# araffin/srl-zoo

Measured on AMD Instinct MI355X. Metric: images/sec (224x224x3) AE+VAE train step, higher is better.
Workload: dtype f32; 1 GPU; synthetic 224x224x3 obs, --losses autoencoder, custom_cnn, state-dim 200, bs=256 per GPU (512 frames fwd+bwd per step per GPU), Adam lr 0.005, normalised fp32 observations resident in HBM; global_batch=256, parallelism=dp1, rccl_ranks=1, devices=1

## Files before the change

include/srlz.h:

```cpp
#ifndef SRLZ_H
#define SRLZ_H

#include <stddef.h>
#include <stdint.h>

#ifdef __cplusplus
extern "C" {
#endif

typedef void* srlz_stream_t;

enum srlz_status {
  SRLZ_OK = 0,
  SRLZ_ERR_BAD_DESC = -1,
  SRLZ_ERR_WORKSPACE = -2,
  SRLZ_ERR_HIP = -3,
  SRLZ_ERR_NULL = -4
};

#define SRLZ_ABI_VERSION 104
int srlz_version(void);
const char* srlz_last_error(void);
int srlz_device_cus(void);

// ... 4 lines not shown
  int ksize;
  int stride;
  int pad;
  int transposed;
  int groups;
} srlz_conv64_desc;

size_t srlz_conv64_packed_floats(void);
int srlz_conv64_pack_weights(const float* w_ref, float* wpack_fwd, float* wpack_bwd,
                             const srlz_conv64_desc* d, srlz_stream_t stream);
int srlz_conv64_fwd_tiles(const srlz_conv64_desc* d);
int srlz_conv64_fwd(const float* x, const float* wpack_fwd, const float* bias, float* y, float* stats_partial,
                    const float* x_bnp, const srlz_conv64_desc* d, srlz_stream_t stream);
typedef struct {
  const float* y;
  const float* bnp;
  const float* sums;
  long long count;
  int training;
  float* dy_out;
} srlz_bn_bwd_operand;
int srlz_conv64_bwd_data(const float* dy, const float* wpack_bwd, float* dx, const srlz_bn_bwd_operand* dy_bn,
                         const srlz_conv64_desc* d, srlz_stream_t stream);
struct srlz_pool_desc_s;
int srlz_conv64_bwd_data_tiles(const srlz_conv64_desc* d);
int srlz_conv64_bwd_data_pool_sums(const float* dy, const float* wpack_bwd, float* dx, const float* pooled, const float* pool_bnp,
                                   const float* pool_y, const uint8_t* pool_argmax, const struct srlz_pool_desc_s* pd,
                                   float* bn_bwd_partial, const srlz_conv64_desc* d, srlz_stream_t stream);
int srlz_conv64_bwd_fused_supported(const srlz_conv64_desc* d);
int srlz_conv64_gather_pipe_supported(const srlz_conv64_desc* d, int backward_data);
int srlz_conv64_scatter_pipe_supported(const srlz_conv64_desc* d, int backward_data);
size_t srlz_conv64_bwd_fused_workspace(const srlz_conv64_desc* d);
int srlz_conv64_bwd_fused_bn_rows(const srlz_conv64_desc* d);
int srlz_conv64_bwd_fused_workgroups(const srlz_conv64_desc* d);
int srlz_conv64_bwd_fused(const float* x, const float* x_bnp, const float* dy, const srlz_bn_bwd_operand* dy_bn,
                          const float* wpack_bwd, float* dx, float* dw_ref, float* dbias ,
                          float* x_bn_bwd_partial , void* ws, size_t ws_bytes, const srlz_conv64_desc* d,
                          srlz_stream_t stream);
int srlz_conv64_wino_supported(const srlz_conv64_desc* d);
size_t srlz_conv64_wino_packed_floats(void);
int srlz_conv64_wino_pack_weights(const float* w_ref, float* upack_fwd, float* upack_bwd, srlz_stream_t stream);
int srlz_conv64_wino_tiles(const srlz_conv64_desc* d);
int srlz_conv64_wino_fwd(const float* x, const float* upack_fwd, const float* bias , float* y,
                         float* stats_partial , const float* x_bnp ,
                         const srlz_conv64_desc* d, srlz_stream_t stream);
int srlz_conv64_wino_bwd_data(const float* dy, const float* upack_bwd, float* dx, const srlz_conv64_desc* d, srlz_stream_t stream);
int srlz_conv64_wino_bwd_data_rows(const srlz_conv64_desc* d);
int srlz_conv64_wino_bwd_data_pool_sums(const float* dy, const float* upack_bwd, float* dx, const float* pooled, const float* pool_bnp,
                                        const float* pool_y, const uint8_t* pool_argmax, const struct srlz_pool_desc_s* pd,
                                        float* bn_bwd_partial, const srlz_conv64_desc* d, srlz_stream_t stream);
size_t srlz_conv64_wino_bwd_weight_workspace(const srlz_conv64_desc* d);
int srlz_conv64_wino_bwd_weight(const float* x, const float* dy, float* dw_ref, void* ws, size_t ws_bytes, const srlz_conv64_desc* d,
                                srlz_stream_t stream);
size_t srlz_conv64_bwd_weight_workspace(const srlz_conv64_desc* d);
int srlz_conv64_bwd_weight(const float* x, const float* dy, float* dw_ref, float* dbias, const float* x_bnp ,
                           const srlz_bn_bwd_operand* dy_bn ,
                           void* ws, size_t ws_bytes, const srlz_conv64_desc* d, srlz_stream_t stream);
int srlz_conv64_bwd_weight_plan(const srlz_conv64_desc* d, int has_x_bnp, int has_dy_bn, int out[4]);

typedef struct {
  int n, hi, wi, ho, wo;
  int cin, cout;
  int ksize, stride, pad;
  int groups;
} srlz_convn_desc;
size_t srlz_convn_packed_floats(const srlz_convn_desc* d);
int srlz_convn_pack_weights(const float* w_ref, float* wpack, const srlz_convn_desc* d, srlz_stream_t stream);
int srlz_convn_fwd_tiles(const srlz_convn_desc* d);
int srlz_convn_fwd(const float* x, const float* wpack, float* y, float* stats_partial, const float* x_bnp,
                   const srlz_convn_desc* d, srlz_stream_t stream);

typedef struct {
  int n;
  int c;
  int himg, wimg;
  int hf, wf;
  int kind;
  int groups;
} srlz_skinny_desc;

int srlz_skinny_tiles(const srlz_skinny_desc* d);
int srlz_conv1_workgroups(const srlz_skinny_desc* d);
int srlz_conv1_buffer_staging_supported(const srlz_skinny_desc* d);
int srlz_conv1_fwd(const float* x_nchw, const float* w_ref, float* y_nhwc, float* stats_partial,
                   const srlz_skinny_desc* d, srlz_stream_t stream);
int srlz_conv1_fwd_u8(const uint8_t* x_u8, const float* norm_lut, const float* w_ref, float* y_nhwc, float* stats_partial,
                      const srlz_skinny_desc* d, srlz_stream_t stream);
size_t srlz_skinny_bwd_weight_workspace(const srlz_skinny_desc* d);
int srlz_conv1_bwd_data(const float* dy_nhwc, const float* w_ref, float* dx_nchw, const srlz_skinny_desc* d,
                        srlz_stream_t stream);
int srlz_conv1_bwd_weight(const float* x_nchw, const float* dy_nhwc, float* dw_ref, void* ws, size_t ws_bytes,
                          const srlz_skinny_desc* d, srlz_stream_t stream);
int srlz_conv1_bwd_weight_fused(const float* x_nchw, const float* y_nhwc, const float* bnp, const uint8_t* argmax,
                                const float* dpooled, const float* sums, int training, float* dw_ref, void* ws,
                                size_t ws_bytes, const srlz_skinny_desc* d, const struct srlz_pool_desc_s* pd,
                                srlz_stream_t stream);
int srlz_conv1_bwd_weight_fused_u8(const uint8_t* x_u8, const float* norm_lut, const float* y_nhwc, const float* bnp,
                                   const uint8_t* argmax, const float* dpooled, const float* sums, int training, float* dw_ref,
                                   void* ws, size_t ws_bytes, const srlz_skinny_desc* d, const struct srlz_pool_desc_s* pd,
                                   srlz_stream_t stream);
int srlz_convT_out_fwd(const float* x_nhwc, const float* w_ref, const float* bias, float* y_nchw,
                       const float* x_bnp , const srlz_skinny_desc* d,
                       srlz_stream_t stream);
int srlz_convT_out_bwd_data(const float* dy_nchw, const float* w_ref, float* dx_nhwc, const float* x_raw,
                            const float* x_bnp, float* bn_bwd_partial, const srlz_skinny_desc* d, srlz_stream_t stream);
int srlz_convT_out_bwd_weight(const float* x_nhwc, const float* dy_nchw, float* dw_ref, float* dbias,
// ... 358 lines not shown
```

srl-zoo_amd/csrc/wino.hip:

```cpp
#include "common.h"

namespace {

typedef float f32x2 __attribute__((ext_vector_type(2)));
typedef unsigned u32x2 __attribute__((ext_vector_type(2)));

constexpr int WN_THREADS = 256;
constexpr int WN_TP = 32;
constexpr int WN_CHUNK = 16 * 4 * 64 * 4;
constexpr int WN_VCHUNK = 16 * 4 * WN_TP * 4;
constexpr int WN_VCOMP = 4 * WN_TP * 4;
constexpr unsigned WN_DROP = 0x80000000u;

struct WinoProg {
  int N, G;
  int H, W;
  int PA, PB;
  int ppi, ppg, tpg;
  unsigned mPPI, mPB;
  int sPPI, sPB;
  long long gstride;
};

__global__ void conv64_wino_pack_kernel(const float* __restrict__ w_ref, float* __restrict__ uf, float* __restrict__ ub) {
  const int id = blockIdx.x * blockDim.x + threadIdx.x;
  if (id >= 64 * 64) return;
  const int e = id & 3, m = (id >> 2) & 63, gq = (id >> 8) & 3, p = id >> 10;
  const int k = 16 * p + 4 * gq + e;
#pragma unroll
  for (int dir = 0; dir < 2; ++dir) {
    float* out = dir ? ub : uf;
    if (!out) continue;
    float gk[3][3];
#pragma unroll
    for (int ky = 0; ky < 3; ++ky)
#pragma unroll
      for (int kx = 0; kx < 3; ++kx)
        gk[ky][kx] = dir ? w_ref[((k * 64 + m) * 3 + (2 - ky)) * 3 + (2 - kx)] : w_ref[((m * 64 + k) * 3 + ky) * 3 + kx];
    float t[3][4];
#pragma unroll
    for (int ky = 0; ky < 3; ++ky) {
      t[ky][0] = gk[ky][0];
      t[ky][1] = 0.5f * (gk[ky][0] + gk[ky][1] + gk[ky][2]);
      t[ky][2] = 0.5f * (gk[ky][0] - gk[ky][1] + gk[ky][2]);
      t[ky][3] = gk[ky][2];
    }
#pragma unroll
    for (int nu = 0; nu < 4; ++nu) {
      const float u0 = t[0][nu];
      const float u1 = 0.5f * (t[0][nu] + t[1][nu] + t[2][nu]);
      const float u2 = 0.5f * (t[0][nu] - t[1][nu] + t[2][nu]);
      const float u3 = t[2][nu];
      const float u[4] = {u0, u1, u2, u3};
// ... 484 lines not shown
  const int wave = tid >> 6;
  const int q = lane >> 3, cpair = wave * 8 + (lane & 7);
  const int tw = (((q >> 2) * 2 + ((q >> 1) & 1)) * 64 + 2 * cpair) * 2 + (q & 1);
  const int ch = wave & 1, cq = wave >> 1, l31 = lane & 31, h = lane >> 5;
  const int tz = cq * 4 * WG_COMP + (h * 64 + 32 * ch + l31) * 2, tv = cq * 4 * WG_COMP + (h * 64 + l31) * 2;

  const long long tfl = (long long)P.N * P.H * P.W * 64;
  const __amdgpu_buffer_rsrc_t xb = raw_buffer(x - (P.W + 1) * 64, (unsigned)(tfl * 4) + (unsigned)(P.W + 1) * 256u);
  const __amdgpu_buffer_rsrc_t gb = raw_buffer(dy, (unsigned)(tfl * 4));

  f32x16 acc[4][2];
#pragma unroll
  for (int c = 0; c < 4; ++c)
#pragma unroll
    for (int b = 0; b < 2; ++b)
#pragma unroll
      for (int r = 0; r < 16; ++r) acc[c][b][r] = 0.f;

  const int s0 = slice * P.spw;
  int s1 = s0 + P.spw;
  if (s1 > P.stages) s1 = P.stages;
  WinoWgradRaw rw;
  WinoWgradPatch wp;
  if (s0 < s1) {
    wg_patch(wp, P, s0 * WG_SP + q, cpair);
    wg_request<S>(rw, wp, xb, gb, P.W);
    wg_land<S>(rw, smem + tw, smem + WG_OP + tw);
    wg_patch(wp, P, (s0 + 1) * WG_SP + q, cpair);
    wg_request<S>(rw, wp, xb, gb, P.W);
    for (int s = s0; s < s1; ++s) {
      const int par = (s - s0) & 1;
      float* cur = smem + par * 2 * WG_OP;
      float* nxt = smem + (par ^ 1) * 2 * WG_OP;
      __syncthreads();
      wg_land<S>(rw, nxt + tw, nxt + WG_OP + tw);
      wg_patch(wp, P, (s + 2) * WG_SP + q, cpair);
      wg_request<S>(rw, wp, xb, gb, P.W);
      __builtin_amdgcn_sched_barrier(0);
      wg_mfma_stage(acc, cur + tz, cur + WG_OP + tv);
    }
  }
  float* out = wpart + (size_t)blockIdx.x * (8 * 4096);
#pragma unroll
  for (int c = 0; c < 4; ++c)
#pragma unroll
    for (int b = 0; b < 2; ++b)
#pragma unroll
      for (int r = 0; r < 16; ++r) {
        const int co = 32 * ch + (r & 3) + 8 * (r >> 2) + 4 * h;
        out[((cq * 4 + c) * 64 + co) * 64 + 32 * b + l31] = acc[c][b][r];
      }
}

__global__ __launch_bounds__(256, 2) void conv64_wino_wgrad_kernel(const float* __restrict__ x, const float* __restrict__ dy,
                                                                   float* __restrict__ wpart, const WinoWgradProg P) {
  extern __shared__ __attribute__((aligned(16))) unsigned char smem_raw[];
  float* smem = (float*)smem_raw;
  const int xcd = blockIdx.x & 7, wi = blockIdx.x >> 3, wpx = gridDim.x >> 3;
  const int slice = xcd * (wpx >> 1) + (wi >> 1);
  if (wi & 1) wg_body<1>(x, dy, wpart, P, smem, slice);
  else wg_body<0>(x, dy, wpart, P, smem, slice);
}

__global__ __launch_bounds__(256) void conv64_wino_wgrad_reduce_a(const float* __restrict__ wpart, double* __restrict__ mid, int nwg, int per) {
  const int id = blockIdx.x * 256 + threadIdx.x;
  const int chunk = blockIdx.y;
  const int comp = id >> 12, rest = id & 4095;
  const int xi = comp >> 2, nu = comp & 3;
  const int half = nu >> 1, local = xi * 2 + (nu & 1);
  double t = 0.0;
  const int npair = nwg >> 1;
  for (int k = chunk * per; k < (chunk + 1) * per && k < npair; ++k) {
    const int b = ((k >> 3) * 2 + half) * 8 + (k & 7);
    t += (double)wpart[(size_t)b * (8 * 4096) + local * 4096 + rest];
  }
  mid[((size_t)chunk * 16 + comp) * 4096 + rest] = t;
}

__global__ __launch_bounds__(256) void conv64_wino_wgrad_reduce_b(const double* __restrict__ mid, int chunks, float* __restrict__ dw_ref) {
  __shared__ double m[16][17];
  const int comp = threadIdx.x >> 4, pr = threadIdx.x & 15;
  const int id = blockIdx.x * 16 + pr;
  double t = 0.0;
  for (int k = 0; k < chunks; ++k) t += mid[((size_t)k * 16 + comp) * 4096 + id];
  m[pr][comp] = t;
  __syncthreads();
  if (threadIdx.x < 144) {
    const int p2 = threadIdx.x / 9, tap = threadIdx.x - p2 * 9, ky = tap / 3, kx = tap - ky * 3;
    double r[4];
#pragma unroll
    for (int nu = 0; nu < 4; ++nu) {
      const double m0 = m[p2][nu], m1 = m[p2][4 + nu], m2 = m[p2][8 + nu], m3 = m[p2][12 + nu];
      r[nu] = ky == 0 ? m0 + 0.5 * (m1 + m2) : ky == 1 ? 0.5 * (m1 - m2) : 0.5 * (m1 + m2) + m3;
    }
    const double v = kx == 0 ? r[0] + 0.5 * (r[1] + r[2]) : kx == 1 ? 0.5 * (r[1] - r[2]) : 0.5 * (r[1] + r[2]) + r[3];
    dw_ref[(blockIdx.x * 16 + p2) * 9 + tap] = (float)v;
  }
}

constexpr int WG_CHUNKS = 8;

int wino_wgrad_program(WinoWgradProg* P, const srlz_conv64_desc* d, int* grid) {
  WinoProg F;
  if (wino_program(&F, d)) return 1;
  const long long total = (long long)d->n * F.ppi;
  if ((long long)d->n * d->hi * d->wi * 256 + (long long)(d->wi + 1) * 256 >= 0x7FFF0000LL || total + 64 >= (1LL << 31)) return 1;
  P->N = d->n; P->H = d->hi; P->W = d->wi; P->PA = F.PA; P->PB = F.PB; P->ppi = F.ppi;
  P->total = (int)total;
  P->stages = (int)((total + WG_SP - 1) / WG_SP);
  P->mPPI = F.mPPI; P->sPPI = F.sPPI; P->mPB = F.mPB; P->sPB = F.sPB;
  int g = 2 * srlz_device_cus();
  g = (g + 15) & ~15;
  while (g > 16 && (g >> 1) * 4 > P->stages) g -= 16;
  const int slices = g >> 1;
  P->spw = (P->stages + slices - 1) / slices;
  *grid = g;
  return 0;
}

}

extern "C" int srlz_conv64_wino_supported(const srlz_conv64_desc* d) {
  WinoProg P;
  return wino_program(&P, d) ? 0 : 1;
}

extern "C" size_t srlz_conv64_wino_packed_floats(void) { return (size_t)4 * WN_CHUNK; }

extern "C" int srlz_conv64_wino_pack_weights(const float* w_ref, float* upack_fwd, float* upack_bwd, srlz_stream_t stream) {
  SRLZ_REQUIRE(w_ref && (upack_fwd || upack_bwd), SRLZ_ERR_NULL, "conv64_wino_pack_weights: null pointer");
  SRLZ_LAUNCH(conv64_wino_pack_kernel, dim3(16), dim3(256), 0, as_stream(stream), w_ref, upack_fwd, upack_bwd);
  return 0;
}

extern "C" int srlz_conv64_wino_tiles(const srlz_conv64_desc* d) {
  WinoProg P;
  if (wino_program(&P, d)) return -1;
  return P.G * P.tpg;
}

static int wino_launch(const float* x, const float* upack, const float* bias, float* y, float* partial, const WinoProg& P,
                       const PoolSum* ps, const float* x_bnp, srlz_stream_t stream) {
  const int ntiles = P.G * P.tpg;
  int grid = 2 * srlz_device_cus();
  if (ntiles < grid) grid = ntiles;
  grid = (grid + 7) & ~7;
  const size_t lds = (size_t)2 * WN_VCHUNK * 4 + 2 * WN_TP * 4;
  const PoolSum none = SRLZ_NO_POOLSUM;
  hipStream_t st = as_stream(stream);
  if (ps) {
    SRLZ_MAX_LDS((conv64_wino_kernel<true, false>), lds);
    SRLZ_LAUNCH((conv64_wino_kernel<true, false>), dim3(grid), dim3(WN_THREADS), lds, st, x, upack, bias, y, partial, P, ntiles, *ps, x_bnp);
  } else if (x_bnp) {
    SRLZ_MAX_LDS((conv64_wino_kernel<false, true>), lds);
    SRLZ_LAUNCH((conv64_wino_kernel<false, true>), dim3(grid), dim3(WN_THREADS), lds, st, x, upack, bias, y, partial, P, ntiles, none, x_bnp);
  } else {
    SRLZ_MAX_LDS((conv64_wino_kernel<false, false>), lds);
    SRLZ_LAUNCH((conv64_wino_kernel<false, false>), dim3(grid), dim3(WN_THREADS), lds, st, x, upack, bias, y, partial, P, ntiles, none, x_bnp);
  }
  if (ps) {
    SRLZ_LAUNCH(conv64_wino_poolsum_zero_scale_kernel, dim3(WN_ZBLOCKS, P.G), dim3(256), 0, st, (const float*)y, *ps, partial, P.N, P.H,
                P.W, P.gstride, P.tpg + WN_ZBLOCKS, P.tpg);
  }
  return 0;
}

extern "C" int srlz_conv64_wino_bwd_data_rows(const srlz_conv64_desc* d) {
  WinoProg P;
  if (wino_program(&P, d)) return -1;
  return P.G * (P.tpg + WN_ZBLOCKS);
}

extern "C" int srlz_conv64_wino_fwd(const float* x, const float* upack, const float* bias, float* y, float* stats_partial,
                                    const float* x_bnp, const srlz_conv64_desc* d, srlz_stream_t stream) {
  SRLZ_REQUIRE(x && upack && y, SRLZ_ERR_NULL, "conv64_wino_fwd: null pointer");
  WinoProg P;
  SRLZ_REQUIRE(wino_program(&P, d) == 0, SRLZ_ERR_BAD_DESC,
               "conv64_wino_fwd: 3x3 stride 1 pad 1 on even sizes only (ask srlz_conv64_wino_supported)");
  return wino_launch(x, upack, bias, y, stats_partial, P, nullptr, x_bnp, stream);
}

extern "C" int srlz_conv64_wino_bwd_data(const float* dy, const float* upack_bwd, float* dx, const srlz_conv64_desc* d, srlz_stream_t stream) {
  SRLZ_REQUIRE(dy && upack_bwd && dx, SRLZ_ERR_NULL, "conv64_wino_bwd_data: null pointer");
  WinoProg P;
  SRLZ_REQUIRE(wino_program(&P, d) == 0, SRLZ_ERR_BAD_DESC,
               "conv64_wino_bwd_data: 3x3 stride 1 pad 1 on even sizes only (ask srlz_conv64_wino_supported)");
  return wino_launch(dy, upack_bwd, nullptr, dx, nullptr, P, nullptr, nullptr, stream);
}

extern "C" int srlz_conv64_wino_bwd_data_pool_sums(const float* dy, const float* upack_bwd, float* dx, const float* pooled,
                                                   const float* pool_bnp, const float* pool_y, const uint8_t* pool_argmax,
                                                   const srlz_pool_desc* pd, float* bn_bwd_partial, const srlz_conv64_desc* d,
                                                   srlz_stream_t stream) {
  SRLZ_REQUIRE(dy && upack_bwd && dx && pooled && pool_bnp && pool_y && pool_argmax && pd && bn_bwd_partial, SRLZ_ERR_NULL,
               "conv64_wino_bwd_data_pool_sums: null pointer");
  WinoProg P;
  SRLZ_REQUIRE(wino_program(&P, d) == 0, SRLZ_ERR_BAD_DESC,
               "conv64_wino_bwd_data_pool_sums: 3x3 stride 1 pad 1 on even sizes only (ask srlz_conv64_wino_supported)");
  SRLZ_REQUIRE(pd->n == d->n && pd->hp == d->hi && pd->wp == d->wi && !pd->out_nchw && (pd->groups > 1 ? pd->groups : 1) == P.G,
               SRLZ_ERR_BAD_DESC, "conv64_wino_bwd_data_pool_sums: the pooled map [%d,%d,%d] is not this layer's input [%d,%d,%d]", pd->n, pd->hp,
               pd->wp, d->n, d->hi, d->wi);
  const PoolSum ps = {pooled, pool_bnp, pool_y, pool_argmax, (long long)(pd->n / P.G) * pd->h * pd->w * 64, pd->h, pd->w, pd->pool_pad};
  return wino_launch(dy, upack_bwd, nullptr, dx, bn_bwd_partial, P, &ps, nullptr, stream);
}

extern "C" size_t srlz_conv64_wino_bwd_weight_workspace(const srlz_conv64_desc* d) {
  WinoWgradProg P;
  int grid;
  if (wino_wgrad_program(&P, d, &grid)) return 0;
  return (size_t)grid * 8 * 4096 * sizeof(float) + (size_t)WG_CHUNKS * 16 * 4096 * sizeof(double);
}

extern "C" int srlz_conv64_wino_bwd_weight(const float* x, const float* dy, float* dw_ref, void* ws, size_t ws_bytes,
                                           const srlz_conv64_desc* d, srlz_stream_t stream) {
  SRLZ_REQUIRE(x && dy && dw_ref && ws, SRLZ_ERR_NULL, "conv64_wino_bwd_weight: null pointer");
  WinoWgradProg P;
  int grid;
  SRLZ_REQUIRE(wino_wgrad_program(&P, d, &grid) == 0, SRLZ_ERR_BAD_DESC,
               "conv64_wino_bwd_weight: 3x3 stride 1 pad 1 on even sizes only (ask srlz_conv64_wino_supported)");
  const size_t part_bytes = (size_t)grid * 8 * 4096 * sizeof(float);
  SRLZ_REQUIRE(ws_bytes >= part_bytes + (size_t)WG_CHUNKS * 16 * 4096 * sizeof(double), SRLZ_ERR_WORKSPACE,
               "conv64_wino_bwd_weight: workspace too small (%zu bytes)", ws_bytes);
  hipStream_t st = as_stream(stream);
  const size_t lds = (size_t)4 * WG_OP * 4;
  SRLZ_MAX_LDS(conv64_wino_wgrad_kernel, lds);
  SRLZ_LAUNCH(conv64_wino_wgrad_kernel, dim3(grid), dim3(256), lds, st, x, dy, (float*)ws, P);
  double* mid = (double*)((char*)ws + part_bytes);
  const int npair = grid >> 1, per = (npair + WG_CHUNKS - 1) / WG_CHUNKS;
  SRLZ_LAUNCH(conv64_wino_wgrad_reduce_a, dim3(65536 / 256, WG_CHUNKS), dim3(256), 0, st, (const float*)ws, mid, grid, per);
  SRLZ_LAUNCH(conv64_wino_wgrad_reduce_b, dim3(256), dim3(256), 0, st, (const double*)mid, WG_CHUNKS, dw_ref);
  return 0;
}
```

srl-zoo_amd/srlz/_cabi.py:

```python
import ctypes
import os
from ctypes import c_int, c_longlong, c_ulonglong, c_float, c_double, c_void_p, c_size_t, c_char_p, POINTER, Structure

_HERE = os.path.dirname(os.path.abspath(__file__))
LIB_PATH = os.path.join(_HERE, "libsrlz_hip.so")


ABI_VERSION = 104


class SrlzError(RuntimeError):
    pass


class Conv64Desc(Structure):
    _fields_ = [("n", c_int), ("hi", c_int), ("wi", c_int), ("ho", c_int), ("wo", c_int), ("ksize", c_int),
                ("stride", c_int), ("pad", c_int), ("transposed", c_int), ("groups", c_int)]


class SkinnyDesc(Structure):
    _fields_ = [("n", c_int), ("c", c_int), ("himg", c_int), ("wimg", c_int), ("hf", c_int), ("wf", c_int),
                ("kind", c_int), ("groups", c_int)]


# ... 20 lines not shown


class InferBlockDesc(Structure):
    _fields_ = [("n", c_int), ("c_in", c_int), ("hi", c_int), ("wi", c_int), ("kind", c_int), ("pool_pad", c_int),
                ("out_nchw", c_int), ("stride_n", c_longlong), ("stride_c", c_longlong), ("stride_y", c_longlong),
                ("stride_x", c_longlong)]


INFER_IN, INFER_MID, INFER_LAST = 0, 1, 2


class InferDecDesc(Structure):
    _fields_ = [("n", c_int), ("c_in", c_int), ("c_out", c_int), ("hi", c_int), ("wi", c_int), ("kind", c_int), ("out_u8", c_int),
                ("bgr", c_int), ("in_stride_n", c_longlong), ("in_stride_c", c_longlong), ("in_stride_y", c_longlong),
                ("in_stride_x", c_longlong), ("out_stride_n", c_longlong), ("out_stride_c", c_longlong),
                ("out_stride_y", c_longlong), ("out_stride_x", c_longlong)]


INFER_DEC_FIRST, INFER_DEC_MID, INFER_DEC_OUT = 0, 1, 2

P = c_void_p
_BO = POINTER(BnBwdOperand)
_C64 = POINTER(Conv64Desc)
_SK = POINTER(SkinnyDesc)
_PD = POINTER(PoolDesc)
_CN = POINTER(ConvNDesc)
_IB = POINTER(InferBlockDesc)
_ID = POINTER(InferDecDesc)

_PROTOS = {
    "srlz_version": (c_int, []),
    "srlz_last_error": (c_char_p, []),
    "srlz_device_cus": (c_int, []),
    "srlz_conv64_packed_floats": (c_size_t, []),
    "srlz_conv64_pack_weights": (c_int, [P, P, P, _C64, P]),
    "srlz_conv64_fwd_tiles": (c_int, [_C64]),
    "srlz_conv64_fwd": (c_int, [P, P, P, P, P, P, _C64, P]),
    "srlz_conv64_bwd_data": (c_int, [P, P, P, _BO, _C64, P]),
    "srlz_conv64_bwd_weight_workspace": (c_size_t, [_C64]),
    "srlz_conv64_bwd_fused_supported": (c_int, [_C64]),
    "srlz_conv64_gather_pipe_supported": (c_int, [_C64, c_int]),
    "srlz_conv64_scatter_pipe_supported": (c_int, [_C64, c_int]),
    "srlz_conv64_bwd_fused_workspace": (c_size_t, [_C64]),
    "srlz_conv64_bwd_fused": (c_int, [P, P, P, _BO, P, P, P, P, P, P, c_size_t, _C64, P]),
    "srlz_conv64_bwd_fused_bn_rows": (c_int, [_C64]),
    "srlz_conv64_wino_supported": (c_int, [_C64]),
    "srlz_conv64_wino_packed_floats": (c_size_t, []),
    "srlz_conv64_wino_pack_weights": (c_int, [P, P, P, P]),
    "srlz_conv64_wino_tiles": (c_int, [_C64]),
    "srlz_conv64_wino_fwd": (c_int, [P, P, P, P, P, P, _C64, P]),
    "srlz_conv64_wino_bwd_data": (c_int, [P, P, P, _C64, P]),
    "srlz_conv64_wino_bwd_weight_workspace": (c_size_t, [_C64]),
    "srlz_conv64_wino_bwd_weight": (c_int, [P, P, P, P, c_size_t, _C64, P]),
    "srlz_conv64_wino_bwd_data_rows": (c_int, [_C64]),
    "srlz_conv64_wino_bwd_data_pool_sums": (c_int, [P, P, P, P, P, P, P, _PD, P, _C64, P]),
    "srlz_conv64_bwd_weight": (c_int, [P, P, P, P, P, _BO, P, c_size_t, _C64, P]),
    "srlz_conv64_bwd_weight_plan": (c_int, [_C64, c_int, c_int, POINTER(c_int)]),
    "srlz_conv64_bwd_fused_workgroups": (c_int, [_C64]),
    "srlz_conv1_workgroups": (c_int, [_SK]),
    "srlz_conv1_buffer_staging_supported": (c_int, [_SK]),
    "srlz_debug_conv1_fwd_generic": (c_int, [P, P, P, P, _SK, P]),
    "srlz_debug_conv1_fwd_u8_generic": (c_int, [P, P, P, P, P, _SK, P]),
    "srlz_debug_conv1_bwd_weight_fused_generic": (c_int, [P, P, P, P, P, P, c_int, P, P, c_size_t, _SK, _PD, P]),
    "srlz_debug_conv1_bwd_weight_fused_u8_generic": (c_int, [P, P, P, P, P, P, P, c_int, P, P, c_size_t, _SK, _PD, P]),
    "srlz_convT_out_os_plan": (c_int, [_SK, c_int, POINTER(c_int)]),
    "srlz_conv64_debug_program": (c_int, [_C64, c_int, POINTER(c_int), c_int]),
    "srlz_linear_debug_route": (c_int, [c_int, c_int, c_int, c_int, c_int, P, P, c_int, c_size_t, POINTER(c_int)]),
    "srlz_debug_placement": (c_int, [P, c_int, c_int, c_int, P]),
    "srlz_debug_mfma_peak": (c_int, [P, c_int, c_int, P]),
    "srlz_debug_mfma_valu": (c_int, [P, c_int, c_int, c_int, c_int, c_int, P]),
    "srlz_convn_packed_floats": (c_size_t, [_CN]),
    "srlz_convn_pack_weights": (c_int, [P, P, _CN, P]),
    "srlz_convn_fwd_tiles": (c_int, [_CN]),
    "srlz_convn_fwd": (c_int, [P, P, P, P, P, _CN, P]),
    "srlz_bn_finalize_chunks_workspace": (c_size_t, [c_int, c_int]),
    "srlz_bn_finalize_chunks": (c_int, [P, c_int, c_int, c_int, c_longlong, P, P, c_float, c_float, P, P, P, P, P, c_size_t, P]),
    "srlz_bn_eval_params_chunks": (c_int, [P, P, P, P, c_float, c_int, P, P]),
    "srlz_bn_add_relu": (c_int, [P, P, P, P, P, c_longlong, c_int, c_int, P]),
    "srlz_avgpool_nhwc": (c_int, [P, P, c_int, c_int, c_int, P]),
    "srlz_prelu_fwd": (c_int, [P, P, P, c_longlong, P]),
    "srlz_prelu_bwd": (c_int, [P, P, P, P, P, c_longlong, P]),
    "srlz_triplet_fwd": (c_int, [P, P, P, c_int, c_int, c_float, P, P, P]),
    "srlz_triplet_bwd": (c_int, [P, P, P, P, P, c_int, c_int, P, P, P, P]),
    "srlz_skinny_tiles": (c_int, [_SK]),
    "srlz_conv64_bwd_data_tiles": (c_int, [_C64]),
    "srlz_conv64_bwd_data_pool_sums": (c_int, [P, P, P, P, P, P, P, _PD, P, _C64, P]),
    "srlz_conv1_fwd": (c_int, [P, P, P, P, _SK, P]),
    "srlz_conv1_fwd_u8": (c_int, [P, P, P, P, P, _SK, P]),
    "srlz_conv1_bwd_weight_fused_u8": (c_int, [P, P, P, P, P, P, P, c_int, P, P, c_size_t, _SK, _PD, P]),
    "srlz_convT_out_fwd_loss_u8": (c_int, [P, P, P, P, P, P, P, P, P, _SK, P]),
    "srlz_normalize_lut": (c_int, [P, P]),
    "srlz_normalize_u8_planar": (c_int, [P, P, P, c_int, c_int, c_longlong, P]),
    "srlz_copy_frames_u8": (c_int, [P, P, c_longlong, P, P, c_longlong, c_int, c_longlong, P]),
    "srlz_copy_frames_u8_strided": (c_int, [P, P, c_longlong, c_longlong, c_longlong, P, P, c_longlong, c_longlong, c_longlong, c_int,
                                            c_longlong, P]),
    "srlz_occlude_frames_u8": (c_int, [P, P, c_longlong, P, P, P, c_int, c_int, c_int, c_int, P]),
    "srlz_skinny_bwd_weight_workspace": (c_size_t, [_SK]),
    "srlz_conv1_bwd_weight": (c_int, [P, P, P, P, c_size_t, _SK, P]),
    "srlz_conv1_bwd_data": (c_int, [P, P, P, _SK, P]),
    "srlz_conv1_bwd_weight_fused": (c_int, [P, P, P, P, P, P, c_int, P, P, c_size_t, _SK, _PD, P]),
    "srlz_bn_relu_pool_bwd_sums": (c_int, [P, P, P, P, P, P, P, P, P, c_size_t, _PD, P]),
    "srlz_convT_out_fwd": (c_int, [P, P, P, P, P, _SK, P]),
    "srlz_convT_out_bwd_data": (c_int, [P, P, P, P, P, P, _SK, P]),
    "srlz_bn_bwd_finalize_partials": (c_int, [P, c_int, c_int, P, P, P, P, c_size_t, P]),
    "srlz_convT_out_bwd_weight": (c_int, [P, P, P, P, P, P, c_size_t, _SK, P]),
    "srlz_convT_out_bwd_fused_supported": (c_int, [_SK]),
# ... 88 lines not shown
    "srlz_param_norms_grad": (c_int, [P, P, P, c_int, c_int, P, P, c_float, P]),
    "srlz_fold_grads": (c_int, [P, P, c_longlong, c_int, P]),
    "srlz_comm_unique_id_bytes": (c_size_t, []),
    "srlz_comm_unique_id": (c_int, [P]),
    "srlz_comm_init": (c_int, [P, c_int, c_int]),
    "srlz_comm_world": (c_int, []),
    "srlz_comm_allreduce_f32": (c_int, [P, c_longlong, P]),
    "srlz_comm_destroy": (c_int, []),
    "srlz_adam_step": (c_int, [P, P, P, P, c_longlong, c_double, c_double, c_double, c_double, c_int, c_float, P]),
    "srlz_adam_step_dev": (c_int, [P, P, P, P, c_longlong, c_double, c_double, c_double, c_double, P, P, c_float, P]),
    "srlz_infer_block_supported": (c_int, [_IB]),
    "srlz_infer_block_out_dims": (c_int, [_IB, POINTER(c_int), POINTER(c_int), POINTER(c_int), POINTER(c_int)]),
    "srlz_infer_tile": (c_int, []),
    "srlz_infer_packed_floats": (c_longlong, [c_int, c_int]),
    "srlz_infer_pack_weights": (c_int, [P, P, c_int, c_int, P]),
    "srlz_infer_block": (c_int, [P, P, P, P, P, _IB, P]),
    "srlz_infer_dec_supported": (c_int, [_ID]),
    "srlz_infer_dec_out_dims": (c_int, [_ID, POINTER(c_int), POINTER(c_int)]),
    "srlz_infer_dec_tile": (c_int, [c_int]),
    "srlz_infer_dec_packed_floats": (c_longlong, [c_int, c_int]),
    "srlz_infer_dec_pack_weights": (c_int, [P, P, c_int, c_int, P]),
    "srlz_infer_dec_block": (c_int, [P, P, P, P, P, _ID, P]),
    "srlz_infer_dec_out": (c_int, [P, P, P, P, _ID, P]),
    "srlz_rollout_supported": (c_int, [c_int, c_int, c_int, c_int]),
    "srlz_rollout_tile": (c_int, []),
    "srlz_rollout": (c_int, [P, P, c_longlong, P, P, P, P, P, P, P, P, P, P, P, P, c_int, c_int, c_int, c_int, c_int, c_int, c_int,
                             c_float, P]),
    "srlz_plan_supported": (c_int, [c_int, c_int, c_int, c_int, c_int, c_int]),
    "srlz_plan_workspace": (c_size_t, [c_int, c_int, c_int, c_int]),
    "srlz_plan_cem": (c_int, [P, P, P, P, P, P, P, P, P, P, c_longlong, P, P, P, P, P, P, c_size_t, c_int, c_int, c_int, c_int, c_int,
                              c_int, c_int, c_int, c_int, c_int, c_float, c_ulonglong, P]),
    "srlz_rollout_goal_supported": (c_int, [c_int, c_int, c_int, c_int, c_int]),
    "srlz_rollout_goal": (c_int, [P, P, c_longlong, P, P, P, P, P, P, P, P, P, P, P, P, c_int, c_int, c_int, c_int, c_int, c_int, c_int,
                                  c_float, P, c_longlong, c_float, c_int, P, P]),
    "srlz_plan_goal_supported": (c_int, [c_int, c_int, c_int, c_int, c_int, c_int, c_int]),
    "srlz_plan_goal_workspace": (c_size_t, [c_int, c_int, c_int, c_int]),
    "srlz_plan_cem_goal": (c_int, [P, P, P, P, P, P, P, P, P, P, c_longlong, P, P, P, P, P, P, c_size_t, c_int, c_int, c_int, c_int,
                                   c_int, c_int, c_int, c_int, c_int, c_int, c_float, c_ulonglong, P, c_longlong, c_float, c_int, P]),
    "srlz_beam_supported": (c_int, [c_int, c_int, c_int, c_int, c_int, c_int, c_int]),
    "srlz_beam_workspace": (c_size_t, [c_int, c_int, c_int, c_int, c_int]),
    "srlz_beam_leaves": (c_int, [c_int, c_int, c_int]),
    "srlz_beam_search": (c_int, [P, P, P, P, P, P, P, P, P, P, P, P, P, P, c_size_t, c_int, c_int, c_int, c_int, c_int, c_int, c_int,
                                 c_float, P, c_longlong, c_float, c_int, P]),
    "srlz_horizon_supported": (c_int, [c_int, c_int, c_int, c_int, c_int]),
    "srlz_horizon_rows": (c_int, [P, P, P, P, P, P, P, P, P, P, P, P, P, P, P, P, c_int, c_int, c_int, c_int, c_int, c_int, c_int, P]),
    "srlz_horizon_sums": (c_int, [P, P, P, P, P, P, c_int, c_int, P, P, P, P, P]),
}

_NOT_STATUS = {"srlz_version", "srlz_device_cus", "srlz_conv64_fwd_tiles", "srlz_skinny_tiles", "srlz_convn_fwd_tiles",
               "srlz_convT_out_bwd_fused_tiles", "srlz_convT_out_fwd_loss_workgroups", "srlz_conv64_bwd_fused_supported", "srlz_conv64_gather_pipe_supported",
               "srlz_conv64_scatter_pipe_supported",
               "srlz_convT_out_bwd_fused_supported",
               "srlz_conv64_bwd_data_tiles", "srlz_conv64_bwd_fused_bn_rows", "srlz_conv64_wino_supported", "srlz_conv64_wino_packed_floats",
               "srlz_conv64_wino_tiles", "srlz_conv64_wino_bwd_data_rows",
               "srlz_conv64_debug_program", "srlz_comm_world", "srlz_dense_supported",
               "srlz_dense_out_fwd_loss_workgroups", "srlz_reward_probe_chunk_rows", "srlz_infer_block_supported",
               "srlz_infer_tile", "srlz_conv64_bwd_fused_workgroups", "srlz_conv1_workgroups",
               "srlz_conv1_buffer_staging_supported", "srlz_infer_dec_supported", "srlz_infer_dec_tile", "srlz_rollout_supported",
               "srlz_rollout_tile", "srlz_plan_supported", "srlz_rollout_goal_supported", "srlz_plan_goal_supported",
               "srlz_horizon_supported", "srlz_beam_supported", "srlz_beam_leaves"}

EXPORTED = sorted(_PROTOS.keys())


def _load():
    if not os.path.exists(LIB_PATH):
        raise SrlzError(
            "libsrlz_hip.so not found at %s — build it with `python -c 'import __graft_entry__ as g; g.build()'` "
            "(or `make -C srl-zoo_amd/csrc`). There is no CPU fallback for the srl-zoo_amd hot path." % LIB_PATH)
    lib = ctypes.CDLL(LIB_PATH)
    for name, (res, args) in _PROTOS.items():
        fn = getattr(lib, name)
        fn.restype = res
        fn.argtypes = args
    got = lib.srlz_version()
    if got != ABI_VERSION:
        raise SrlzError("libsrlz_hip.so at %s reports ABI version %d, these bindings are written for %d (include/srlz.h "
                        "SRLZ_ABI_VERSION): rebuild with `make -C srl-zoo_amd/csrc`" % (LIB_PATH, got, ABI_VERSION))
    return lib


_lib = _load()


def error_text():
    return _lib.srlz_last_error().decode("utf-8", "replace")


_DEBUG_SYNC = bool(os.environ.get("SRLZ_SYNC"))


def _wrap(name):
    fn = getattr(_lib, name)
    if _PROTOS[name][0] is c_int and name not in _NOT_STATUS:
        def call(*a):
            rc = fn(*a)
            if rc != 0:
                raise SrlzError("%s failed (%d): %s" % (name, rc, error_text()))
            if _DEBUG_SYNC:
                import torch
                torch.cuda.synchronize()
            return rc
        call.__name__ = name
        return call
    return fn


# ... 14 lines not shown
```

Before: 45960 images/s.

## Fuse Winograd weight-grad split pair into one 512-thread workgroup with shared patch table

The old weight-gradient kernel ran two 256-thread workgroups per slice, each handling half of the Winograd components and each re-deriving patch addresses. The new default kernel merges them into one 512-thread workgroup: four waves transform x tiles and four waves transform dy tiles into shared LDS, one wave builds a small ring of patch-offset tables ahead of use, and every wave runs MFMA on both component halves. This aims to cut duplicate input loads, address arithmetic and launch count, and to overlap loads with MFMA through explicit scheduling barriers. The cost is more LDS per block and more accumulator registers, which may lower occupancy. The reduction kernel gains a flag for the new partial layout, and the old path stays available as a debug fallback when LDS opt-in is too small.

```diff
diff --git a/include/srlz.h b/include/srlz.h
--- a/include/srlz.h
+++ b/include/srlz.h
@@ -80,6 +80,9 @@
 size_t srlz_conv64_wino_bwd_weight_workspace(const srlz_conv64_desc* d);
 int srlz_conv64_wino_bwd_weight(const float* x, const float* dy, float* dw_ref, void* ws, size_t ws_bytes, const srlz_conv64_desc* d,
                                 srlz_stream_t stream);
+int srlz_debug_conv64_wino_bwd_weight_split(const float* x, const float* dy, float* dw_ref, void* ws, size_t ws_bytes,
+                                            const srlz_conv64_desc* d, srlz_stream_t stream);
+int srlz_debug_conv64_wino_bwd_weight_route(const srlz_conv64_desc* d);
 size_t srlz_conv64_bwd_weight_workspace(const srlz_conv64_desc* d);
 int srlz_conv64_bwd_weight(const float* x, const float* dy, float* dw_ref, float* dbias, const float* x_bnp ,
                            const srlz_bn_bwd_operand* dy_bn ,
diff --git a/srl-zoo_amd/csrc/wino.hip b/srl-zoo_amd/csrc/wino.hip
--- a/srl-zoo_amd/csrc/wino.hip
+++ b/srl-zoo_amd/csrc/wino.hip
@@ -1,4 +1,5 @@
 #include "common.h"
+#include <type_traits>
 
 namespace {
 
@@ -589,8 +590,8 @@
       }
 }
 
-__global__ __launch_bounds__(256, 2) void conv64_wino_wgrad_kernel(const float* __restrict__ x, const float* __restrict__ dy,
-                                                                   float* __restrict__ wpart, const WinoWgradProg P) {
+__global__ __launch_bounds__(256, 2) void conv64_wino_wgrad_split_kernel(const float* __restrict__ x, const float* __restrict__ dy,
+                                                                         float* __restrict__ wpart, const WinoWgradProg P) {
   extern __shared__ __attribute__((aligned(16))) unsigned char smem_raw[];
   float* smem = (float*)smem_raw;
   const int xcd = blockIdx.x & 7, wi = blockIdx.x >> 3, wpx = gridDim.x >> 3;
@@ -599,7 +600,222 @@
   else wg_body<0>(x, dy, wpart, P, smem, slice);
 }
 
-__global__ __launch_bounds__(256) void conv64_wino_wgrad_reduce_a(const float* __restrict__ wpart, double* __restrict__ mid, int nwg, int per) {
+typedef unsigned u32x4 __attribute__((ext_vector_type(4)));
+
+constexpr int W1_THREADS = 512;
+constexpr int W1_OP = 16 * WG_COMP;
+constexpr int W1_TSLOTS = 4;
+constexpr int W1_TENT = 12;
+constexpr size_t W1_LDS = (size_t)4 * W1_OP * 4 + (size_t)W1_TSLOTS * WG_SP * W1_TENT * 4;
+
+__device__ __forceinline__ void w1_table(unsigned* slot, const WinoWgradProg& P, int stage, int q) {
+  WinoWgradPatch wp;
+  wg_patch(wp, P, stage * WG_SP + q, 0);
+  u32x4* e = (u32x4*)(slot + q * W1_TENT);
+  e[0] = u32x4{wp.vtop, wp.vmid, wp.vbot, wp.vmid};
+  e[1] = u32x4{wp.lef ? wp.vtop : WN_DROP, wp.lef ? wp.vmid : WN_DROP, wp.lef ? wp.vbot : WN_DROP, WN_DROP};
+  e[2] = u32x4{wp.rig ? wp.vtop : WN_DROP, wp.rig ? wp.vmid : WN_DROP, wp.rig ? wp.vbot : WN_DROP, WN_DROP};
+}
+
+struct W1Entry { u32x4 m, l, r; };
+
+template <int ROLE>
+__device__ __forceinline__ void w1_entry(W1Entry& t, const unsigned* ent) {
+  if (ROLE == 0) { t.m = *(const u32x4*)ent; t.l = *(const u32x4*)(ent + 4); t.r = *(const u32x4*)(ent + 8); }
+  else t.m[1] = ent[1];
+}
+
+template <int ROLE>
+__device__ __forceinline__ void w1_request(f32x2 (&d)[ROLE == 0 ? 16 : 4], const W1Entry& t, unsigned cp8, __amdgpu_buffer_rsrc_t xb,
+                                           __amdgpu_buffer_rsrc_t gb, int W) {
+  if (ROLE == 0) {
+#pragma unroll
+    for (int r = 0; r < 4; ++r)
+#pragma unroll
+      for (int c = 0; c < 4; ++c) {
+        const u32x4 cls = c == 0 ? t.l : c == 3 ? t.r : t.m;
+        const unsigned off = (r == 0 ? cls[0] : r == 3 ? cls[2] : cls[1]) + cp8;
+        const u32x2 v = __builtin_amdgcn_raw_buffer_load_b64(xb, off + (unsigned)(c * 256), r * W * 256, 0);
+        d[r * 4 + c] = f32x2{__uint_as_float(v[0]), __uint_as_float(v[1])};
+      }
+  } else {
+    const unsigned off = t.m[1] + cp8;
+#pragma unroll
+    for (int i = 0; i < 2; ++i)
+#pragma unroll
+      for (int j = 0; j < 2; ++j) {
+        const u32x2 v = __builtin_amdgcn_raw_buffer_load_b64(gb, off + (unsigned)(j * 256), i * W * 256, 0);
+        d[i * 2 + j] = f32x2{__uint_as_float(v[0]), __uint_as_float(v[1])};
+      }
+  }
+}
+
+template <int ROLE>
+__device__ __forceinline__ void w1_land(const f32x2 (&d)[ROLE == 0 ? 16 : 4], float* __restrict__ Ow) {
+  int two = 2;
+  asm volatile("" : "+v"(two));
+  float* __restrict__ Ow1 = Ow + two;
+#pragma unroll
+  for (int S = 0; S < 2; ++S) {
+    f32x2 o[2][4];
+    if (ROLE == 0) {
+      f32x2 e[4][2];
+#pragma unroll
+      for (int r = 0; r < 4; ++r) {
+        if (S == 0) { e[r][0] = d[r * 4 + 0] - d[r * 4 + 2]; e[r][1] = d[r * 4 + 1] + d[r * 4 + 2]; }
+        else        { e[r][0] = d[r * 4 + 2] - d[r * 4 + 1]; e[r][1] = d[r * 4 + 1] - d[r * 4 + 3]; }
+      }
+#pragma unroll
+      for (int j = 0; j < 2; ++j) {
+        o[j][0] = e[0][j] - e[2][j]; o[j][1] = e[1][j] + e[2][j]; o[j][2] = e[2][j] - e[1][j]; o[j][3] = e[1][j] - e[3][j];
+      }
+    } else {
+      f32x2 t[2][2];
+#pragma unroll
+      for (int i = 0; i < 2; ++i) {
+        if (S == 0) { t[i][0] = d[i * 2]; t[i][1] = d[i * 2] + d[i * 2 + 1]; }
+        else        { t[i][0] = d[i * 2] - d[i * 2 + 1]; t[i][1] = -d[i * 2 + 1]; }
+      }
+#pragma unroll
+      for (int j = 0; j < 2; ++j) {
+        o[j][0] = t[0][j]; o[j][1] = t[0][j] + t[1][j]; o[j][2] = t[0][j] - t[1][j]; o[j][3] = -t[1][j];
+      }
+    }
+#pragma unroll
+    for (int ch = 0; ch < 2; ++ch)
+#pragma unroll
+      for (int j = 0; j < 2; ++j)
+#pragma unroll
+        for (int xi = 0; xi < 4; ++xi) (ch ? Ow1 : Ow)[(xi * 4 + 2 * S + j) * WG_COMP] = o[j][xi][ch];
+  }
+}
+
+struct W1Frag { f32x2 z[2][2], v[2][2]; };
+
+__device__ __forceinline__ void w1_read(W1Frag& f, const float* __restrict__ Zp, const float* __restrict__ Vp) {
+#pragma unroll
+  for (int j = 0; j < 2; ++j)
+#pragma unroll
+    for (int b = 0; b < 2; ++b) {
+      f.z[j][b] = *(const f32x2*)(Zp + j * 256 + b * 64);
+      f.v[j][b] = *(const f32x2*)(Vp + j * 256 + b * 64);
+    }
+}
+
+__device__ __forceinline__ void w1_mfma_comp(f32x16 (&acc)[2][2], const W1Frag& f) {
+#pragma unroll
+  for (int j = 0; j < 2; ++j)
+#pragma unroll
+    for (int e = 0; e < 2; ++e)
+#pragma unroll
+      for (int bo = 0; bo < 2; ++bo)
+#pragma unroll
+        for (int bi = 0; bi < 2; ++bi)
+          acc[bo][bi] = __builtin_amdgcn_mfma_f32_32x32x2f32(f.z[j][bo][e], f.v[j][bi][e], acc[bo][bi], 0, 0, 0);
+}
+
+template <int ROLE>
+__device__ __forceinline__ void w1_body(const float* __restrict__ x, const float* __restrict__ dy, float* __restrict__ wpart,
+                                        const WinoWgradProg& P, float* smem, int slice, int wave) {
+  const int tid = threadIdx.x;
+  int lane = tid & 63;
+  asm volatile("" : "+v"(lane));
+  const int q = lane >> 3, cpair = (wave & 3) * 8 + (lane & 7);
+  const unsigned cp8 = (unsigned)cpair * 8u;
+  const int tw = (ROLE == 0 ? W1_OP : 0) + (((q >> 2) * 2 + ((q >> 1) & 1)) * 64 + 2 * cpair) * 2 + (q & 1);
+  unsigned* tab = (unsigned*)(smem + 4 * W1_OP);
+  const bool builder = ROLE == 1 && wave == 4 && lane < WG_SP;
+  const int l31 = lane & 31, h = lane >> 5;
+  const int tm = wave * 2 * WG_COMP + (h * 64 + l31) * 2;
+
+  const long long tfl = (long long)P.N * P.H * P.W * 64;
+  const __amdgpu_buffer_rsrc_t xb = raw_buffer(x - (P.W + 1) * 64, (unsigned)(tfl * 4) + (unsigned)(P.W + 1) * 256u);
+  const __amdgpu_buffer_rsrc_t gb = raw_buffer(dy, (unsigned)(tfl * 4));
+
+  f32x16 acc[2][2][2];
+#pragma unroll
+  for (int c = 0; c < 2; ++c)
+#pragma unroll
+    for (int bo = 0; bo < 2; ++bo)
+#pragma unroll
+      for (int bi = 0; bi < 2; ++bi)
+#pragma unroll
+        for (int r = 0; r < 16; ++r) acc[c][bo][bi][r] = 0.f;
+
+  const int s0 = slice * P.spw;
+  int s1 = s0 + P.spw;
+  if (s1 > P.stages) s1 = P.stages;
+  if (s0 < s1) {
+    f32x2 raw[ROLE == 0 ? 16 : 4];
+    W1Entry te;
+    W1Frag f1;
+    if (builder) {
+#pragma unroll
+      for (int i = 0; i < 3; ++i) w1_table(tab + i * WG_SP * W1_TENT, P, s0 + i, lane);
+    }
+    __syncthreads();
+    w1_entry<ROLE>(te, tab + q * W1_TENT);
+    w1_request<ROLE>(raw, te, cp8, xb, gb, P.W);
+    w1_land<ROLE>(raw, smem + tw);
+    w1_entry<ROLE>(te, tab + (WG_SP + q) * W1_TENT);
+    w1_request<ROLE>(raw, te, cp8, xb, gb, P.W);
+    auto stage = [&](auto first, int s) {
+      constexpr bool FIRST = decltype(first)::value;
+      const int k = s - s0;
+      float* cur = smem + (k & 1) * 2 * W1_OP;
+      float* nxt = smem + ((k & 1) ^ 1) * 2 * W1_OP;
+      __syncthreads();
+      W1Frag f0;
+      w1_read(f0, cur + tm, cur + W1_OP + tm);
+      w1_entry<ROLE>(te, tab + (((k + 2) & (W1_TSLOTS - 1)) * WG_SP + q) * W1_TENT);
+      __builtin_amdgcn_sched_barrier(0);
+      if (ROLE == 1 && !FIRST) w1_mfma_comp(acc[1], f1);
+      w1_land<ROLE>(raw, nxt + tw);
+      w1_request<ROLE>(raw, te, cp8, xb, gb, P.W);
+      if (builder) w1_table(tab + ((k + 3) & (W1_TSLOTS - 1)) * WG_SP * W1_TENT, P, s + 3, lane);
+      if (ROLE == 0 && !FIRST) w1_mfma_comp(acc[1], f1);
+      __builtin_amdgcn_sched_barrier(0);
+      w1_read(f1, cur + tm + WG_COMP, cur + W1_OP + tm + WG_COMP);
+      w1_mfma_comp(acc[0], f0);
+#pragma unroll
+      for (int i = 0; i < 8; ++i) {
+        __builtin_amdgcn_sched_group_barrier(0x100, 1, 0);
+        __builtin_amdgcn_sched_group_barrier(0x008, 1, 0);
+      }
+      __builtin_amdgcn_sched_group_barrier(0x008, 8, 0);
+      __builtin_amdgcn_sched_barrier(0);
+    };
+    stage(std::true_type{}, s0);
+    for (int s = s0 + 1; s < s1; ++s) stage(std::false_type{}, s);
+    w1_mfma_comp(acc[1], f1);
+  }
+  float* out = wpart + (size_t)blockIdx.x * (16 * 4096) + (size_t)wave * (2 * 4096);
+#pragma unroll
+  for (int c = 0; c < 2; ++c)
+#pragma unroll
+    for (int bo = 0; bo < 2; ++bo)
+#pragma unroll
+      for (int bi = 0; bi < 2; ++bi)
+#pragma unroll
+        for (int r = 0; r < 16; ++r) {
+          const int co = 32 * bo + (r & 3) + 8 * (r >> 2) + 4 * h;
+          out[(c * 64 + co) * 64 + 32 * bi + l31] = acc[c][bo][bi][r];
+        }
+}
+
+__global__ __launch_bounds__(W1_THREADS, 2) void conv64_wino_wgrad_kernel(const float* __restrict__ x, const float* __restrict__ dy,
+                                                                          float* __restrict__ wpart, const WinoWgradProg P) {
+  extern __shared__ __attribute__((aligned(16))) unsigned char smem_raw[];
+  float* smem = (float*)smem_raw;
+  const int xcd = blockIdx.x & 7, wi = blockIdx.x >> 3, wpx = gridDim.x >> 3;
+  const int slice = xcd * wpx + wi;
+  const int wave = __builtin_amdgcn_readfirstlane(threadIdx.x >> 6);
+  if (wave < 4) w1_body<0>(x, dy, wpart, P, smem, slice, wave);
+  else w1_body<1>(x, dy, wpart, P, smem, slice, wave);
+}
+
+__global__ __launch_bounds__(256) void conv64_wino_wgrad_reduce_a(const float* __restrict__ wpart, double* __restrict__ mid, int nwg, int per,
+                                                                  int onepass) {
   const int id = blockIdx.x * 256 + threadIdx.x;
   const int chunk = blockIdx.y;
   const int comp = id >> 12, rest = id & 4095;
@@ -609,7 +825,7 @@
   const int npair = nwg >> 1;
   for (int k = chunk * per; k < (chunk + 1) * per && k < npair; ++k) {
     const int b = ((k >> 3) * 2 + half) * 8 + (k & 7);
-    t += (double)wpart[(size_t)b * (8 * 4096) + local * 4096 + rest];
+    t += (double)(onepass ? wpart[(size_t)k * (16 * 4096) + comp * 4096 + rest] : wpart[(size_t)b * (8 * 4096) + local * 4096 + rest]);
   }
   mid[((size_t)chunk * 16 + comp) * 4096 + rest] = t;
 }
@@ -653,6 +869,18 @@
   P->spw = (P->stages + slices - 1) / slices;
   *grid = g;
   return 0;
+}
+
+bool wino_wgrad_onepass(const WinoWgradProg& P, int grid) {
+  static int lds_optin = -1;
+  if (lds_optin < 0) {
+    int dev = 0, v = 0, w = 0;
+    if (hipGetDevice(&dev) != hipSuccess || hipDeviceGetAttribute(&v, hipDeviceAttributeMaxSharedMemoryPerBlock, dev) != hipSuccess) v = 0;
+    if (v && hipDeviceGetAttribute(&w, hipDeviceAttributeSharedMemPerBlockOptin, dev) != hipSuccess) w = 0;
+    (void)hipGetLastError();
+    lds_optin = v > w ? v : w;
+  }
+  return (size_t)lds_optin >= W1_LDS && (grid & 15) == 0 && P.stages > 0;
 }
 
 }
@@ -748,23 +976,46 @@
   return (size_t)grid * 8 * 4096 * sizeof(float) + (size_t)WG_CHUNKS * 16 * 4096 * sizeof(double);
 }
 
-extern "C" int srlz_conv64_wino_bwd_weight(const float* x, const float* dy, float* dw_ref, void* ws, size_t ws_bytes,
-                                           const srlz_conv64_desc* d, srlz_stream_t stream) {
-  SRLZ_REQUIRE(x && dy && dw_ref && ws, SRLZ_ERR_NULL, "conv64_wino_bwd_weight: null pointer");
+static int wino_wgrad_launch(const char* who, bool allow_onepass, const float* x, const float* dy, float* dw_ref, void* ws, size_t ws_bytes,
+                             const srlz_conv64_desc* d, srlz_stream_t stream) {
+  SRLZ_REQUIRE(x && dy && dw_ref && ws, SRLZ_ERR_NULL, "%s: null pointer", who);
   WinoWgradProg P;
   int grid;
   SRLZ_REQUIRE(wino_wgrad_program(&P, d, &grid) == 0, SRLZ_ERR_BAD_DESC,
-               "conv64_wino_bwd_weight: 3x3 stride 1 pad 1 on even sizes only (ask srlz_conv64_wino_supported)");
+               "%s: 3x3 stride 1 pad 1 on even sizes only (ask srlz_conv64_wino_supported)", who);
   const size_t part_bytes = (size_t)grid * 8 * 4096 * sizeof(float);
   SRLZ_REQUIRE(ws_bytes >= part_bytes + (size_t)WG_CHUNKS * 16 * 4096 * sizeof(double), SRLZ_ERR_WORKSPACE,
-               "conv64_wino_bwd_weight: workspace too small (%zu bytes)", ws_bytes);
+               "%s: workspace too small (%zu bytes)", who, ws_bytes);
   hipStream_t st = as_stream(stream);
-  const size_t lds = (size_t)4 * WG_OP * 4;
-  SRLZ_MAX_LDS(conv64_wino_wgrad_kernel, lds);
-  SRLZ_LAUNCH(conv64_wino_wgrad_kernel, dim3(grid), dim3(256), lds, st, x, dy, (float*)ws, P);
+  const int onepass = allow_onepass && wino_wgrad_onepass(P, grid) ? 1 : 0;
+  if (onepass) {
+    SRLZ_MAX_LDS(conv64_wino_wgrad_kernel, W1_LDS);
+    SRLZ_LAUNCH(conv64_wino_wgrad_kernel, dim3(grid >> 1), dim3(W1_THREADS), W1_LDS, st, x, dy, (float*)ws, P);
+  } else {
+    const size_t lds = (size_t)4 * WG_OP * 4;
+    SRLZ_MAX_LDS(conv64_wino_wgrad_split_kernel, lds);
+    SRLZ_LAUNCH(conv64_wino_wgrad_split_kernel, dim3(grid), dim3(256), lds, st, x, dy, (float*)ws, P);
+  }
   double* mid = (double*)((char*)ws + part_bytes);
   const int npair = grid >> 1, per = (npair + WG_CHUNKS - 1) / WG_CHUNKS;
-  SRLZ_LAUNCH(conv64_wino_wgrad_reduce_a, dim3(65536 / 256, WG_CHUNKS), dim3(256), 0, st, (const float*)ws, mid, grid, per);
+  SRLZ_LAUNCH(conv64_wino_wgrad_reduce_a, dim3(65536 / 256, WG_CHUNKS), dim3(256), 0, st, (const float*)ws, mid, grid, per, onepass);
   SRLZ_LAUNCH(conv64_wino_wgrad_reduce_b, dim3(256), dim3(256), 0, st, (const double*)mid, WG_CHUNKS, dw_ref);
   return 0;
 }
+
+extern "C" int srlz_conv64_wino_bwd_weight(const float* x, const float* dy, float* dw_ref, void* ws, size_t ws_bytes,
+                                           const srlz_conv64_desc* d, srlz_stream_t stream) {
+  return wino_wgrad_launch("conv64_wino_bwd_weight", true, x, dy, dw_ref, ws, ws_bytes, d, stream);
+}
+
+extern "C" int srlz_debug_conv64_wino_bwd_weight_split(const float* x, const float* dy, float* dw_ref, void* ws, size_t ws_bytes,
+                                                       const srlz_conv64_desc* d, srlz_stream_t stream) {
+  return wino_wgrad_launch("debug_conv64_wino_bwd_weight_split", false, x, dy, dw_ref, ws, ws_bytes, d, stream);
+}
+
+extern "C" int srlz_debug_conv64_wino_bwd_weight_route(const srlz_conv64_desc* d) {
+  WinoWgradProg P;
+  int grid;
+  if (wino_wgrad_program(&P, d, &grid)) return -1;
+  return wino_wgrad_onepass(P, grid) ? 1 : 0;
+}
diff --git a/srl-zoo_amd/srlz/_cabi.py b/srl-zoo_amd/srlz/_cabi.py
--- a/srl-zoo_amd/srlz/_cabi.py
+++ b/srl-zoo_amd/srlz/_cabi.py
@@ -96,6 +96,8 @@
     "srlz_conv64_wino_bwd_data": (c_int, [P, P, P, _C64, P]),
     "srlz_conv64_wino_bwd_weight_workspace": (c_size_t, [_C64]),
     "srlz_conv64_wino_bwd_weight": (c_int, [P, P, P, P, c_size_t, _C64, P]),
+    "srlz_debug_conv64_wino_bwd_weight_split": (c_int, [P, P, P, P, c_size_t, _C64, P]),
+    "srlz_debug_conv64_wino_bwd_weight_route": (c_int, [_C64]),
     "srlz_conv64_wino_bwd_data_rows": (c_int, [_C64]),
     "srlz_conv64_wino_bwd_data_pool_sums": (c_int, [P, P, P, P, P, P, P, _PD, P, _C64, P]),
     "srlz_conv64_bwd_weight": (c_int, [P, P, P, P, P, _BO, P, c_size_t, _C64, P]),
@@ -290,7 +292,7 @@
                "srlz_conv64_scatter_pipe_supported",
                "srlz_convT_out_bwd_fused_supported",
                "srlz_conv64_bwd_data_tiles", "srlz_conv64_bwd_fused_bn_rows", "srlz_conv64_wino_supported", "srlz_conv64_wino_packed_floats",
-               "srlz_conv64_wino_tiles", "srlz_conv64_wino_bwd_data_rows",
+               "srlz_conv64_wino_tiles", "srlz_conv64_wino_bwd_data_rows", "srlz_debug_conv64_wino_bwd_weight_route",
                "srlz_conv64_debug_program", "srlz_comm_world", "srlz_dense_supported",
                "srlz_dense_out_fwd_loss_workgroups", "srlz_reward_probe_chunk_rows", "srlz_infer_block_supported",
                "srlz_infer_tile", "srlz_conv64_bwd_fused_workgroups", "srlz_conv1_workgroups",
```

Result: no change. 46160 images/s, median of 4 (+0.4%).
